# m1nty/Real-Time-Software-Defined-Radio

Measured on AMD Instinct MI355X. Metric: IQ MSamples/s through RF front-end+mono path; achieved HBM GB/s vs peak, higher is better.
Workload: dtype f32; 1 GPU; RF front end (101-tap LPF, decim 10, atan2 demod) + mono (151-tap LPF, decim 5): configs[1]+[2], one stream per GPU; block_complex=1024000, taps=101, iq=f32, parallelism=independent streams x1

## Files before the change

### real-time-software-defined-radio_amd/csrc/fe_mfma.hip

```cpp
#include <cmath>
#include <cstdlib>

#include "sdr_launch.h"

namespace {

typedef int i4v __attribute__((ext_vector_type(4)));

constexpr float kPiF = 3.14159265358979323846f;
#ifndef SDR_FE_MFMA_ABL
#define SDR_FE_MFMA_ABL 0
#endif
constexpr int kAbl = SDR_FE_MFMA_ABL;
#define SDR_FE_MFMA_WPE 3

constexpr float k2PiF = 6.28318530717958647692f;

struct MfmaFe {
  const unsigned char* iq;
  int64_t n, stride;
  int64_t M, A;
  int bps;
  int64_t total;
  const float* taps;
  float qscale;
  const float* argev;
  const i4v* afr;
  float* audio;
  int64_t audio_stride;
};

constexpr int D = 10, T = 101, TO = 256, OFF = 104;
constexpr int IMG = D * TO + 96;
constexpr int NCH = IMG / 8;
constexpr int NLD = (NCH + 63) / 64;
constexpr int TA = 151, DA = 5, AB = DA * TO, HA = 152, NW = DA * 3 + TA;
static_assert(IMG % 8 == 0 && NLD == 6, "image layout");
static_assert(D * 15 + T - 1 + (OFF - 100 - 0) < 256 && OFF - (T - 1) >= 0, "K = 256 covers the band");

__device__ __forceinline__ void lds_order() { asm volatile("" ::: "memory"); }

__device__ __forceinline__ unsigned bperm(int src_lane, unsigned v) {
  return (unsigned)__builtin_amdgcn_ds_bpermute(src_lane << 2, (int)v);
}

int tap_scale_exp(float hmax) { return (int)std::floor(std::log2((8388608.0 - 65536.0) / (double)hmax)); }

__device__ __forceinline__ int digit(int q, int k) {
  int d = 0;
  for (int j = 0; j <= k; ++j) {
    d = ((q & 0xff) ^ 0x80) - 0x80;
    q = (q - d) >> 8;
  }
  return d;
}

__device__ __forceinline__ void combine_digits(const i4v (&acc)[2][3], float (&yi)[4], float (&yq)[4]) {
#pragma unroll
  for (int i = 0; i < 4; ++i) {
    yi[i] = fmaf((float)acc[0][2][i], 65536.f, (float)(acc[0][1][i] * 256 + acc[0][0][i]));
    yq[i] = fmaf((float)acc[1][2][i], 65536.f, (float)(acc[1][1][i] * 256 + acc[1][0][i]));
  }
}
__device__ __forceinline__ f2v atan2_x2_finite(f2v y, f2v x) {
  const float ax0 = fabsf(x.x), ay0 = fabsf(y.x), ax1 = fabsf(x.y), ay1 = fabsf(y.y);
  const float mn0 = fminf(ax0, ay0), mx0 = fmaxf(ax0, ay0), mn1 = fminf(ax1, ay1), mx1 = fmaxf(ax1, ay1);
  const f2v mn = f2v{mn0, mn1};
  const f2v mxs = f2v{fmaxf(mx0, 1e-30f), fmaxf(mx1, 1e-30f)};
  const f2v rc = f2v{__builtin_amdgcn_rcpf(mxs.x), __builtin_amdgcn_rcpf(mxs.y)};
  f2v a = mn * rc;
  a = __builtin_elementwise_fma(__builtin_elementwise_fma(-mxs, a, mn), rc, a);
  const f2v s = a * a;
  auto c = [](float v) { return f2v{v, v}; };
  f2v r = c(0.002849547192454338f);
  r = __builtin_elementwise_fma(r, s, c(-0.01606736145913601f));
  r = __builtin_elementwise_fma(r, s, c(0.04268963634967804f));
  r = __builtin_elementwise_fma(r, s, c(-0.0750415101647377f));
  r = __builtin_elementwise_fma(r, s, c(0.1064087525010109f));
  r = __builtin_elementwise_fma(r, s, c(-0.1420363187789917f));
  r = __builtin_elementwise_fma(r, s, c(0.19992618262767792f));
  r = __builtin_elementwise_fma(r, s, c(-0.3333307206630707f));
  r = __builtin_elementwise_fma(r, s, c(1.0f));
  r = r * a;
  float r0 = r.x, r1 = r.y;
  r0 = (ay0 > ax0) ? 1.57079632679489662f - r0 : r0;
  r1 = (ay1 > ax1) ? 1.57079632679489662f - r1 : r1;
  r0 = (x.x < 0.f) ? 3.14159265358979324f - r0 : r0;
  r1 = (x.y < 0.f) ? 3.14159265358979324f - r1 : r1;
  asm volatile("" : "+v"(r0), "+v"(r1));
  r0 = (mx0 == 0.f) ? (__builtin_signbitf(x.x) ? 3.14159265358979324f : 0.f) : r0;
  r1 = (mx1 == 0.f) ? (__builtin_signbitf(x.y) ? 3.14159265358979324f : 0.f) : r1;
  return f2v{copysignf(r0, y.x), copysignf(r1, y.y)};
}
template <bool FINITE>
__device__ __forceinline__ void atan2_4(const float (&y)[4], const float (&x)[4], float (&phi)[4]) {
  const f2v p01 = FINITE ? atan2_x2_finite(f2v{y[0], y[1]}, f2v{x[0], x[1]}) : fast_atan2f_x2(f2v{y[0], y[1]}, f2v{x[0], x[1]});
  const f2v p23 = FINITE ? atan2_x2_finite(f2v{y[2], y[3]}, f2v{x[2], x[3]}) : fast_atan2f_x2(f2v{y[2], y[3]}, f2v{x[2], x[3]});
  phi[0] = p01.x; phi[1] = p01.y; phi[2] = p23.x; phi[3] = p23.y;
}
__device__ __forceinline__ void pk_fma_s(f2v& acc, f2v tap2, const f2v& x2) {
  asm("v_pk_fma_f32 %0, %1, %2, %0" : "+v"(acc) : "s"(tap2), "v"(x2));
}
typedef float f2a4 __attribute__((ext_vector_type(2), aligned(4)));
typedef const __attribute__((address_space(4))) float* cfp4;
typedef const __attribute__((address_space(4))) f2a4* cfp2;

__global__ __launch_bounds__(64) __attribute__((amdgpu_waves_per_eu(SDR_FE_MFMA_WPE))) void fe_mfma_mono_kernel(MfmaFe p) {
  __shared__ __attribute__((aligned(16))) signed char img[2][IMG + 16];
  __shared__ __attribute__((aligned(16))) float dh[HA + AB + 8];

  const int lane = threadIdx.x;
  const int64_t b0 = (int64_t)blockIdx.x * p.total / gridDim.x;
  const int64_t b1 = ((int64_t)blockIdx.x + 1) * p.total / gridDim.x;
  if (b0 >= b1) return;
  const int pl = lane & 15, gl = lane >> 4;

  i4v afr[4][3];
  if (p.afr != nullptr) {
#pragma unroll
    for (int ks = 0; ks < 4; ++ks)
#pragma unroll
      for (int dg = 0; dg < 3; ++dg) afr[ks][dg] = p.afr[(ks * 3 + dg) * 64 + lane];
  } else
#pragma unroll
  for (int ks = 0; ks < 4; ++ks) {
    int w[3][4] = {};
#pragma unroll
    for (int j = 0; j < 16; ++j) {
      const int k = D * pl + OFF - (64 * ks + 16 * gl + j);
      const float h = (k >= 0 && k < T) ? p.taps[k] : 0.f;
      const int q = (int)rintf(h * p.qscale);
#pragma unroll
      for (int dg = 0; dg < 3; ++dg) w[dg][j >> 2] |= (digit(q, dg) & 0xff) << (8 * (j & 3));
    }
#pragma unroll
    for (int dg = 0; dg < 3; ++dg) afr[ks][dg] = i4v{w[dg][0], w[dg][1], w[dg][2], w[dg][3]};
  }
#pragma unroll
  for (int ks = 0; ks < 4; ++ks)
#pragma unroll
    for (int dg = 0; dg < 3; ++dg) asm volatile("" : : "v"(afr[ks][dg]));
  const cfp4 gr = (cfp4)p.argev;

  f4v stg[NLD];
  const unsigned voff = 16u * lane;
  auto n_lo_of = [&](int64_t t) { return (int64_t)TO * D * t - OFF; };
  auto interior = [&](int64_t t) { return n_lo_of(t) >= 0 && n_lo_of(t) + IMG <= p.n; };
  auto base_of = [&](int s, int64_t t) { return p.iq + 2 * ((int64_t)s * p.stride + n_lo_of(t)); };
  constexpr int HC = (IMG - D * TO) / 8;
  static_assert(D * TO / 8 == 5 * 64, "5 new chunks per lane");
  auto load_image = [&](int s, int64_t t, bool halo) {
    const int cf = halo ? HC : 0;
    const unsigned char* base = base_of(s, t) + 16 * cf;
    if (kAbl & 16) return;
    static_for<0, NLD>([&](auto Q) {
      constexpr int q = Q;
      if (lane < NCH - cf - 64 * q) gload16_nt_v<0>(stg[q], voff, base + 1024 * q);
    });
  };
  auto put_chunk = [&](int c, unsigned w0, unsigned w1, unsigned w2, unsigned w3) {
    const unsigned i_lo = __builtin_amdgcn_perm(w1, w0, 0x06040200u) ^ 0x80808080u;
    const unsigned i_hi = __builtin_amdgcn_perm(w3, w2, 0x06040200u) ^ 0x80808080u;
    const unsigned q_lo = __builtin_amdgcn_perm(w1, w0, 0x07050301u) ^ 0x80808080u;
    const unsigned q_hi = __builtin_amdgcn_perm(w3, w2, 0x07050301u) ^ 0x80808080u;
    *reinterpret_cast<uint2*>(&img[0][8 * c]) = make_uint2(i_lo, i_hi);
    *reinterpret_cast<uint2*>(&img[1][8 * c]) = make_uint2(q_lo, q_hi);
  };
  auto store_image = [&](bool halo) {
    asm volatile("s_waitcnt vmcnt(0)" ::: "memory");
    const int cf = halo ? HC : 0;
    if (halo && lane < 2 * HC) {
      const int ch = lane / HC, k = lane - ch * HC;
      const uint2 v = *reinterpret_cast<const uint2*>(&img[ch][D * TO + 8 * k]);
      *reinterpret_cast<uint2*>(&img[ch][8 * k]) = v;
    }
    lds_order();
#pragma unroll
    for (int q = 0; q < NLD; ++q) {
      const int c = cf + lane + 64 * q;
      if (c < NCH) {
        asm volatile("" : "+v"(stg[q]));
        if (!(kAbl & 8))
          put_chunk(c, __float_as_uint(stg[q].x), __float_as_uint(stg[q].y), __float_as_uint(stg[q].z),
                    __float_as_uint(stg[q].w));
      }
    }
  };
  auto build_guarded = [&](int s, int64_t t) {
    const int64_t n_lo = n_lo_of(t);
    const unsigned char* base = base_of(s, t);
    for (int c = lane; c < NCH; c += 64) {
      unsigned w4[4];
#pragma unroll
      for (int e = 0; e < 4; ++e) {
        const int64_t n0 = n_lo + 8 * c + 2 * e;
        const unsigned lo = (n0 >= 0 && n0 < p.n) ? *reinterpret_cast<const unsigned short*>(base + 2 * (8 * c + 2 * e)) : 0x8080u;
        const unsigned hi = (n0 + 1 >= 0 && n0 + 1 < p.n) ? *reinterpret_cast<const unsigned short*>(base + 2 * (8 * c + 2 * e + 1)) : 0x8080u;
        w4[e] = lo | (hi << 16);
      }
      put_chunk(c, w4[0], w4[1], w4[2], w4[3]);
    }
  };

  int s = (int)(b0 / p.bps);
  int64_t t = (b0 - (int64_t)s * p.bps) * DA;
  const int64_t tps = (int64_t)p.bps * DA;
  const bool warm = t > 0;
  if (warm) --t;
  const int64_t U = (b1 - b0) * DA + (warm ? 1 : 0);
  for (int e = lane; e < HA; e += 64) dh[e] = 0.f;
  if (interior(t)) {
    load_image(s, t, false);
    store_image(false);
  } else {
    build_guarded(s, t);
  }
  auto next_s = [&](int s_, int64_t t_) { return t_ + 1 == tps ? s_ + 1 : s_; };
  auto next_t = [&](int64_t t_) { return t_ + 1 == tps ? (int64_t)0 : t_ + 1; };
  int s1 = next_s(s, t);
  int64_t t1 = next_t(t);
  float carry = 0.f;
  float d4[4] = {0.f, 0.f, 0.f, 0.f};

  constexpr int AQ = 4;
  f4v aq[AQ];
  int nq = 0;
  int qs = (int)(b0 / p.bps);
  int qj = (int)(b0 - (int64_t)qs * p.bps);
  auto queue_flush = [&]() __attribute__((always_inline)) {
    static_for<0, AQ>([&](auto K) {
      constexpr int k = K;
      if (k < nq) {
        const int64_t j = (int64_t)TO * qj + 4 * lane;
        float* ao = p.audio + (int64_t)qs * p.audio_stride + j;
        if (j + 4 <= p.A && ((uintptr_t)ao & 15) == 0) {
          *reinterpret_cast<f4v*>(ao) = aq[k];
        } else {
          const float rv[4] = {aq[k].x, aq[k].y, aq[k].z, aq[k].w};
#pragma unroll
          for (int r = 0; r < 4; ++r)
            if (j + r < p.A) ao[r] = rv[r];
        }
        if (++qj == p.bps) { qj = 0; ++qs; }
      }
    });
    nq = 0;
  };
  auto queue_put = [&](const f4v& v) __attribute__((always_inline)) {
    static_for<0, AQ>([&](auto K) {
      if ((int)K == nq) aq[K] = v;
    });
    if (++nq == AQ) queue_flush();
  };

  auto mfma_tile = [&](i4v (&acc)[2][3]) __attribute__((always_inline)) {
    lds_order();
#pragma unroll
    for (int ch = 0; ch < 2; ++ch)
#pragma unroll
      for (int dg = 0; dg < 3; ++dg) acc[ch][dg] = i4v{0, 0, 0, 0};
#pragma unroll
    for (int ks = 0; ks < 4; ++ks) {
      i4v a[3];
#pragma unroll
      for (int dg = 0; dg < 3; ++dg) a[dg] = afr[ks][dg];
      i4v bf[2];
#pragma unroll
      for (int ch = 0; ch < 2; ++ch) bf[ch] = *reinterpret_cast<const i4v*>(&img[ch][160 * pl + 64 * ks + 16 * gl]);
#pragma unroll
      for (int ch = 0; ch < 2; ++ch)
#pragma unroll
        for (int dg = 0; dg < 3; ++dg)
          acc[ch][dg] = (kAbl & 4) ? acc[ch][dg] + bf[ch]
                                   : __builtin_amdgcn_mfma_i32_16x16x64_i8(a[dg], bf[ch], acc[ch][dg], 0, 0, 0);
    }
  };
  auto epilogue = [&](const i4v (&acc)[2][3], int64_t u) __attribute__((always_inline)) {
    float yi[4], yq[4];
    combine_digits(acc, yi, yq);
    float phi[4];
    if (kAbl & 2) {
#pragma unroll
      for (int i = 0; i < 4; ++i) phi[i] = yq[i] * 1e-9f + yi[i] * 1e-9f;
    } else {
      atan2_4<true>(yq, yi, phi);
    }
    const int src = gl > 0 ? lane - 16 : (pl > 0 ? lane + 47 : 63);
    const float left = __uint_as_float(bperm(src, __float_as_uint(phi[3])));
    float prev = (lane == 0) ? carry : left;
    const int64_t mo = (int64_t)TO * t + 16 * pl + 4 * gl;
    float d[4];
#pragma unroll
    for (int i = 0; i < 4; ++i) {
      float dd = phi[i] - prev;
      if (dd > kPiF) dd -= k2PiF;
      else if (dd < -kPiF) dd += k2PiF;
      d[i] = (mo + i == 0) ? phi[i] : dd;
      prev = phi[i];
    }
    carry = __int_as_float(__builtin_amdgcn_readlane(__float_as_int(phi[3]), 63));
    const int o = 16 * pl + 4 * gl;
    const int tb = (int)(t % DA);
    if (warm && u == 0) {
      if (o >= TO - HA) *reinterpret_cast<f4v*>(&dh[HA - TO + o]) = f4v{d[0], d[1], d[2], d[3]};
    } else {
      *reinterpret_cast<f4v*>(&dh[HA + TO * tb + o]) = f4v{d[0], d[1], d[2], d[3]};
#pragma unroll
      for (int i = 0; i < 4; ++i) d4[i] = d[i];
    }
    if (!(kAbl & 1) && !(warm && u == 0) && tb == DA - 1) {
      lds_order();
      const float* aw = dh + (HA - (TA - 1)) + DA * 4 * lane;
      f2v acc[4] = {f2v{0.f, 0.f}, f2v{0.f, 0.f}, f2v{0.f, 0.f}, f2v{0.f, 0.f}};
      static_for<0, NW / 2>([&](auto W2) {
        constexpr int w = 2 * W2;
        const f2v x2 = *reinterpret_cast<const f2v*>(aw + w);
        static_for<0, 4>([&](auto RR) {
          constexpr int j = w - DA * (int)RR;
          if constexpr (j >= -1 && j <= TA - 1) {
            const f2a4 hp = *(cfp2)(gr + j);
            pk_fma_s(acc[RR], f2v{hp.x, hp.y}, x2);
          }
        });
      });
      queue_put(f4v{acc[0].x + acc[0].y, acc[1].x + acc[1].y, acc[2].x + acc[2].y, acc[3].x + acc[3].y});
      lds_order();
      if (o >= TO - HA) *reinterpret_cast<f4v*>(&dh[HA - TO + o]) = f4v{d4[0], d4[1], d4[2], d4[3]};
    }
  };
  auto advance = [&]() __attribute__((always_inline)) {
    s = s1;
    t = t1;
    if (t == 0) {
      lds_order();
      for (int e = lane; e < HA; e += 64) dh[e] = 0.f;
    }
    s1 = next_s(s, t);
    t1 = next_t(t);
  };

  bool staged = U > 1 && interior(t1);
  bool halo = staged && s1 == s && t1 == t + 1 && interior(t);
  if (staged) load_image(s1, t1, halo);
  i4v acc[2][3];
  for (int64_t u = 0; u < U; ++u) {
    const bool more = u + 1 < U;
    mfma_tile(acc);
    if (more) {
      lds_order();
      if (staged) store_image(halo);
      else build_guarded(s1, t1);
      const int s2 = next_s(s1, t1);
      const int64_t t2 = next_t(t1);
      staged = u + 2 < U && interior(t2);
      halo = staged && s2 == s1 && t2 == t1 + 1 && interior(t1);
      if (staged) load_image(s2, t2, halo);
    }
    epilogue(acc, u);
    if (more) advance();
  }
  asm volatile("s_waitcnt vmcnt(0)" ::: "memory");
  queue_flush();
}

template <int T> struct DemodShape;
template <> struct DemodShape<101> { static constexpr int KS = 4, OFF = 104; };
template <> struct DemodShape<151> { static constexpr int KS = 5, OFF = 152; };

struct MfmaDemod {
  const unsigned char* iq;
  int64_t n, stride;
  int64_t M;
  int64_t tps, total;
  const float* taps;
  float qscale;
  const i4v* afr;
  const double* zi_i;
  const double* zi_q;
  int64_t zi_stride;
  const double* prev_phase;
  float* demod;
  int64_t out_stride;
  float* last_phi;
  int* wraps;
  int vec_out;
};

__device__ inline double unwrap_step_f64_m(double dd, int* w) {
  *w = 0;
  if (fabs(dd) < 3.14159265358979323846) return dd;
  constexpr double kPi = 3.14159265358979323846, k2Pi = 6.28318530717958647692;
  double m = fmod(dd + kPi, k2Pi);
  if (m < 0) m += k2Pi;
  double ddmod = m - kPi;
  if (ddmod == -kPi && dd > 0) ddmod = kPi;
  *w = (int)llrint((ddmod - dd) / k2Pi);
  return ddmod;
}

template <int T>
__device__ __forceinline__ float output_phase(const unsigned char* iq_s, int64_t m, const float* taps, float qscale) {
  const int lane = threadIdx.x;
  int acc[2][3] = {};
  for (int k = lane; k < T; k += 64) {
    const int q = (int)rintf(taps[k] * qscale);
    const unsigned short v = *reinterpret_cast<const unsigned short*>(iq_s + 2 * (D * m - k));
    const int xi = (int)(signed char)((v & 0xff) ^ 0x80), xq = (int)(signed char)(((v >> 8) & 0xff) ^ 0x80);
#pragma unroll
    for (int dg = 0; dg < 3; ++dg) {
      const int d = digit(q, dg);
      acc[0][dg] += d * xi;
      acc[1][dg] += d * xq;
    }
  }
#pragma unroll
  for (int ch = 0; ch < 2; ++ch)
#pragma unroll
    for (int dg = 0; dg < 3; ++dg) acc[ch][dg] = wave_sum_i(acc[ch][dg]);
  const float yi = fmaf((float)acc[0][2], 65536.f, (float)(acc[0][1] * 256 + acc[0][0]));
  const float yq = fmaf((float)acc[1][2], 65536.f, (float)(acc[1][1] * 256 + acc[1][0]));
  return fast_atan2f_x2(f2v{yq, yq}, f2v{yi, yi}).x;
}

template <int T>
__global__ __launch_bounds__(64) void fe_mfma_demod_kernel(MfmaDemod p) {
  constexpr int KS = DemodShape<T>::KS, OFF = DemodShape<T>::OFF, K = 64 * KS;
  constexpr int IM = 160 * 15 + K;
  constexpr int NC = IM / 8, NL = (NC + 63) / 64;
  static_assert(IM % 8 == 0 && OFF % 8 == 0 && OFF >= T - 1 && D * 15 + OFF <= K - 1, "image / band layout");
  __shared__ __attribute__((aligned(16))) signed char img[2][IM + 16];

  const int lane = threadIdx.x;
  const int64_t b0 = (int64_t)blockIdx.x * p.total / gridDim.x;
  const int64_t b1 = ((int64_t)blockIdx.x + 1) * p.total / gridDim.x;
  if (b0 >= b1) return;
  const int pl = lane & 15, gl = lane >> 4;

  i4v afr[KS][3];
  if (p.afr != nullptr) {
#pragma unroll
    for (int ks = 0; ks < KS; ++ks)
#pragma unroll
      for (int dg = 0; dg < 3; ++dg) afr[ks][dg] = p.afr[(ks * 3 + dg) * 64 + lane];
  } else
#pragma unroll
  for (int ks = 0; ks < KS; ++ks) {
    int w[3][4] = {};
#pragma unroll
    for (int j = 0; j < 16; ++j) {
      const int k = D * pl + OFF - (64 * ks + 16 * gl + j);
      const float h = (k >= 0 && k < T) ? p.taps[k] : 0.f;
      const int q = (int)rintf(h * p.qscale);
#pragma unroll
      for (int dg = 0; dg < 3; ++dg) w[dg][j >> 2] |= (digit(q, dg) & 0xff) << (8 * (j & 3));
    }
#pragma unroll
    for (int dg = 0; dg < 3; ++dg) afr[ks][dg] = i4v{w[dg][0], w[dg][1], w[dg][2], w[dg][3]};
  }
#pragma unroll
  for (int ks = 0; ks < KS; ++ks)
#pragma unroll
    for (int dg = 0; dg < 3; ++dg) asm volatile("" : : "v"(afr[ks][dg]));

  f4v stg[NL];
  const unsigned voff = 16u * lane;
  auto n_lo_of = [&](int64_t t) { return (int64_t)TO * D * t - OFF; };
  auto interior = [&](int64_t t) { return n_lo_of(t) >= 0 && n_lo_of(t) + IM <= p.n; };
  auto base_of = [&](int s, int64_t t) { return p.iq + 2 * ((int64_t)s * p.stride + n_lo_of(t)); };
  constexpr int HC = (IM - D * TO) / 8;
  static_assert(D * TO / 8 == 5 * 64, "5 new chunks per lane");
  auto load_image = [&](int s, int64_t t, bool halo) {
    const int cf = halo ? HC : 0;
    const unsigned char* base = base_of(s, t) + 16 * cf;
    static_for<0, NL>([&](auto Q) {
      constexpr int q = Q;
      if (lane < NC - cf - 64 * q) gload16_nt_v<0>(stg[q], voff, base + 1024 * q);
    });
  };
  auto put_chunk = [&](int c, unsigned w0, unsigned w1, unsigned w2, unsigned w3) {
    const unsigned i_lo = __builtin_amdgcn_perm(w1, w0, 0x06040200u) ^ 0x80808080u;
    const unsigned i_hi = __builtin_amdgcn_perm(w3, w2, 0x06040200u) ^ 0x80808080u;
    const unsigned q_lo = __builtin_amdgcn_perm(w1, w0, 0x07050301u) ^ 0x80808080u;
    const unsigned q_hi = __builtin_amdgcn_perm(w3, w2, 0x07050301u) ^ 0x80808080u;
    *reinterpret_cast<uint2*>(&img[0][8 * c]) = make_uint2(i_lo, i_hi);
    *reinterpret_cast<uint2*>(&img[1][8 * c]) = make_uint2(q_lo, q_hi);
  };
  bool st1 = false;
  auto store_image = [&](bool halo) {
    if (__builtin_amdgcn_readfirstlane((int)st1)) asm volatile("s_waitcnt vmcnt(1)" ::: "memory");
    else asm volatile("s_waitcnt vmcnt(0)" ::: "memory");
    const int cf = halo ? HC : 0;
    if (halo && lane < 2 * HC) {
      const int ch = lane / HC, k = lane - ch * HC;
      const uint2 v = *reinterpret_cast<const uint2*>(&img[ch][D * TO + 8 * k]);
      *reinterpret_cast<uint2*>(&img[ch][8 * k]) = v;
    }
    lds_order();
#pragma unroll
    for (int q = 0; q < NL; ++q) {
      const int c = cf + lane + 64 * q;
      if (c < NC) {
        asm volatile("" : "+v"(stg[q]));
        put_chunk(c, __float_as_uint(stg[q].x), __float_as_uint(stg[q].y), __float_as_uint(stg[q].z),
                  __float_as_uint(stg[q].w));
      }
    }
  };
  auto build_guarded = [&](int s, int64_t t) {
    const int64_t n_lo = n_lo_of(t);
    const unsigned char* base = base_of(s, t);
    for (int c = lane; c < NC; c += 64) {
      unsigned w4[4];
#pragma unroll
      for (int e = 0; e < 4; ++e) {
        const int64_t n0 = n_lo + 8 * c + 2 * e;
        const unsigned lo = (n0 >= 0 && n0 < p.n) ? *reinterpret_cast<const unsigned short*>(base + 2 * (8 * c + 2 * e)) : 0x8080u;
        const unsigned hi = (n0 + 1 >= 0 && n0 + 1 < p.n) ? *reinterpret_cast<const unsigned short*>(base + 2 * (8 * c + 2 * e + 1)) : 0x8080u;
        w4[e] = lo | (hi << 16);
      }
      put_chunk(c, w4[0], w4[1], w4[2], w4[3]);
    }
  };

  int s = (int)(b0 / p.tps);
  int64_t t = b0 - (int64_t)s * p.tps;
  const int64_t U = b1 - b0;
  float carry = t > 0 ? output_phase<T>(p.iq + 2 * (int64_t)s * p.stride, TO * t - 1, p.taps, p.qscale) : 0.f;
  if (interior(t)) {
    load_image(s, t, false);
    store_image(false);
  } else {
    build_guarded(s, t);
  }
  int s_nx = s;
  int64_t t_nx = t + 1;
  if (t_nx == p.tps) { t_nx = 0; ++s_nx; }
  int wsum = 0;
  const double zscale = (double)p.qscale * 128.0;

  bool staged = U > 1 && interior(t_nx);
  bool halo = staged && s_nx == s && t_nx == t + 1 && interior(t);
  if (staged) load_image(s_nx, t_nx, halo);
  for (int64_t u = 0; u < U; ++u) {
    const bool more = u + 1 < U;
    lds_order();
    i4v acc[2][3];
#pragma unroll
    for (int ch = 0; ch < 2; ++ch)
#pragma unroll
      for (int dg = 0; dg < 3; ++dg) acc[ch][dg] = i4v{0, 0, 0, 0};
#pragma unroll
    for (int ks = 0; ks < KS; ++ks) {
      i4v bf[2];
#pragma unroll
      for (int ch = 0; ch < 2; ++ch) bf[ch] = *reinterpret_cast<const i4v*>(&img[ch][160 * pl + 64 * ks + 16 * gl]);
#pragma unroll
      for (int ch = 0; ch < 2; ++ch)
#pragma unroll
        for (int dg = 0; dg < 3; ++dg)
          acc[ch][dg] = __builtin_amdgcn_mfma_i32_16x16x64_i8(afr[ks][dg], bf[ch], acc[ch][dg], 0, 0, 0);
    }
    if (more) {
      lds_order();
      if (staged) store_image(halo);
      else build_guarded(s_nx, t_nx);
      int s2 = s_nx;
      int64_t t2 = t_nx + 1;
      if (t2 == p.tps) { t2 = 0; ++s2; }
      staged = u + 2 < U && interior(t2);
      halo = staged && s2 == s_nx && t2 == t_nx + 1 && interior(t_nx);
      if (staged) load_image(s2, t2, halo);
    }
    const int64_t mo = (int64_t)TO * t + 16 * pl + 4 * gl;
    float yi[4], yq[4];
    combine_digits(acc, yi, yq);
    if (t == 0 && p.zi_i != nullptr) {
#pragma unroll
      for (int i = 0; i < 4; ++i)
        if (D * (mo + i) < T - 1) {
          yi[i] += (float)(p.zi_i[(int64_t)s * p.zi_stride + D * (mo + i)] * zscale);
          yq[i] += (float)(p.zi_q[(int64_t)s * p.zi_stride + D * (mo + i)] * zscale);
        }
    }
    float phi[4];
    atan2_4<false>(yq, yi, phi);
    const int src = gl > 0 ? lane - 16 : (pl > 0 ? lane + 47 : 63);
    const float left = __uint_as_float(bperm(src, __float_as_uint(phi[3])));
    float prev = (lane == 0) ? carry : left;
    constexpr bool keep = true;
    float d[4];
#pragma unroll
    for (int i = 0; i < 4; ++i) {
      const int64_t m = mo + i;
      int wk = 0;
      if (m == 0) {
        const double ps = p.prev_phase ? p.prev_phase[s] : 0.0;
        d[i] = (float)unwrap_step_f64_m((double)phi[i] - ps, &wk);
      } else {
        float dd = phi[i] - prev;
        if (dd > kPiF) { dd -= k2PiF; wk = -1; }
        else if (dd < -kPiF) { dd += k2PiF; wk = 1; }
        d[i] = dd;
      }
      if (keep && m < p.M) wsum += wk;
      prev = phi[i];
    }
    carry = __int_as_float(__builtin_amdgcn_readlane(__float_as_int(phi[3]), 63));
    if (keep) {
      float* out = p.demod + (int64_t)s * p.out_stride + mo;
      if (p.vec_out && mo + 4 <= p.M) {
        *reinterpret_cast<f4v*>(out) = f4v{d[0], d[1], d[2], d[3]};
      } else {
#pragma unroll
        for (int i = 0; i < 4; ++i)
          if (mo + i < p.M) out[i] = d[i];
      }
      if (p.last_phi != nullptr) {
#pragma unroll
        for (int i = 0; i < 4; ++i)
          if (mo + i == p.M - 1) p.last_phi[s] = phi[i];
      }
    }
    const bool wr = keep && (!more || s_nx != s) && p.wraps != nullptr;
    if (wr) {
      const int w = wave_sum_i(wsum);
      if (lane == 0 && w != 0) atomicAdd(p.wraps + s, w);
      wsum = 0;
    }
    st1 = keep && p.vec_out && t > 0 && (int64_t)TO * t + TO < p.M && !wr;
    if (more) {
      s = s_nx;
      t = t_nx;
      t_nx = t + 1;
      s_nx = s;
      if (t_nx == p.tps) { t_nx = 0; ++s_nx; }
    }
  }
}

template <int T>
hipError_t launch_demod_mfma_t(const FeLaunch& a, hipStream_t st) {
  float hmax = 0.f;
  for (int k = 0; k < T; ++k) hmax = std::max(hmax, std::fabs(a.taps->h[k]));
  if (!(hmax > 0.f) || !std::isfinite(hmax)) return hipErrorInvalidValue;
  const int S = tap_scale_exp(hmax);
  MfmaDemod p{};
  p.iq = static_cast<const unsigned char*>(a.iq);
  p.n = a.n;
  p.stride = a.nstreams > 1 ? a.stride : 0;
  p.M = (a.n + D - 1) / D;
  p.tps = (p.M + TO - 1) / TO;
  p.total = p.tps * a.nstreams;
  if (p.total > 0x7fffffff) return hipErrorInvalidValue;
  p.taps = a.taps_dev;
  p.qscale = std::ldexp(1.0f, S);
  p.afr = reinterpret_cast<const i4v*>(a.afr);
  p.zi_i = a.zi_i;
  p.zi_q = a.zi_q;
  p.zi_stride = a.zi_stride;
  p.prev_phase = a.prev_phase;
  p.demod = a.demod;
  p.out_stride = a.out_stride;
  p.last_phi = a.last_phi;
  p.wraps = a.wraps;
  p.vec_out = ((a.out_stride % 4) == 0 && ((uintptr_t)a.demod % 16) == 0) ? 1 : 0;
  static std::atomic<int> slot_cache[kMaxDevices];
  const int slots = per_device(slot_cache, [] {
    int per = 0;
    if (hipOccupancyMaxActiveBlocksPerMultiprocessor(&per, fe_mfma_demod_kernel<T>, 64, 0) != hipSuccess || per <= 0) per = 1;
    return device_cus() * std::min(per, 12);
  });
  const int64_t run = std::max<int64_t>(1, (p.total + slots - 1) / slots);
  const int64_t grid = std::max<int64_t>(1, (p.total + run - 1) / run);
  hipLaunchKernelGGL(fe_mfma_demod_kernel<T>, dim3((unsigned)grid), dim3(64), 0, st, p);
  return hipGetLastError();
}

}

bool sdr_mfma_fragments(const float* h, int T_, std::vector<int>* out) {
  int KS, OFFT;
  if (T_ == 101) { KS = DemodShape<101>::KS; OFFT = DemodShape<101>::OFF; }
  else if (T_ == 151) { KS = DemodShape<151>::KS; OFFT = DemodShape<151>::OFF; }
  else return false;
  static_assert(DemodShape<101>::KS == 4 && DemodShape<101>::OFF == OFF, "mono and demod kernels share the T = 101 shape");
  float hmax = 0.f;
  for (int k = 0; k < T_; ++k) hmax = std::max(hmax, std::fabs(h[k]));
  if (!(hmax > 0.f) || !std::isfinite(hmax)) return false;
  const float qs = std::ldexp(1.0f, tap_scale_exp(hmax));
  out->assign((size_t)KS * 3 * 64 * 4, 0);
  for (int ks = 0; ks < KS; ++ks)
    for (int lane = 0; lane < 64; ++lane) {
      const int pl = lane & 15, gl = lane >> 4;
      for (int j = 0; j < 16; ++j) {
        const int k = D * pl + OFFT - (64 * ks + 16 * gl + j);
        const float hv = (k >= 0 && k < T_) ? h[k] : 0.f;
        int q = (int)std::rint(hv * qs);
        for (int dg = 0; dg < 3; ++dg) {
          const int d = ((q & 0xff) ^ 0x80) - 0x80;
          q = (q - d) >> 8;
          (*out)[(((size_t)ks * 3 + dg) * 64 + lane) * 4 + (j >> 2)] |= (d & 0xff) << (8 * (j & 3));
        }
      }
    }
  return true;
}

hipError_t sdr_launch_fe_mfma(const FeLaunch& a, hipStream_t st) {
  if (!a.u8 || a.D != D || a.hist != 0 || a.i_ds || a.q_ds || a.demod == nullptr) return hipErrorInvalidValue;
  if (((uintptr_t)a.iq & 15) != 0 || (a.nstreams > 1 && (a.stride % 8) != 0)) return hipErrorInvalidValue;
  if (a.n <= 0 || a.nstreams <= 0) return hipSuccess;
  if (a.T == 101) return launch_demod_mfma_t<101>(a, st);
  if (a.T == 151) return launch_demod_mfma_t<151>(a, st);
  return hipErrorInvalidValue;
}

hipError_t sdr_launch_fe_mono_mfma(const FeLaunch& a, const float* ataps_rev, int TA_, int DA_, float* audio,
                                   int64_t audio_stride, hipStream_t st) {
  if (!a.u8 || a.D != D || a.T != T || TA_ != TA || DA_ != DA || a.hist != 0 || a.zi_i || a.prev_phase || a.demod ||
      a.i_ds || a.last_phi || a.wraps)
    return hipErrorInvalidValue;
  if (((uintptr_t)a.iq & 15) != 0 || (a.nstreams > 1 && (a.stride % 8) != 0)) return hipErrorInvalidValue;
  if (a.n <= 0 || a.nstreams <= 0) return hipSuccess;
  float hmax = 0.f;
  for (int k = 0; k < T; ++k) hmax = std::max(hmax, std::fabs(a.taps->h[k]));
  if (!(hmax > 0.f) || !std::isfinite(hmax)) return hipErrorInvalidValue;
  const int S = tap_scale_exp(hmax);
  MfmaFe p{};
  p.iq = static_cast<const unsigned char*>(a.iq);
  p.n = a.n;
  p.stride = a.nstreams > 1 ? a.stride : 0;
  p.M = (a.n + D - 1) / D;
  p.A = (p.M + DA - 1) / DA;
  p.bps = (int)((p.M + AB - 1) / AB);
  p.total = (int64_t)p.bps * a.nstreams;
  if (p.total > 0x7fffffff) return hipErrorInvalidValue;
  p.taps = a.taps_dev;
  p.qscale = std::ldexp(1.0f, S);
  p.afr = reinterpret_cast<const i4v*>(a.afr);
  p.argev = ataps_rev;
  p.audio = audio;
  p.audio_stride = audio_stride;
  static std::atomic<int> slot_cache[kMaxDevices];
  const int slots = per_device(slot_cache, [] {
    int per = 0;
    if (hipOccupancyMaxActiveBlocksPerMultiprocessor(&per, fe_mfma_mono_kernel, 64, 0) != hipSuccess || per <= 0) per = 1;
    const int cap = 4 * SDR_FE_MFMA_WPE;
    return device_cus() * std::min(per, cap);
  });

  const int64_t grid = std::min<int64_t>(slots, p.total);
  hipLaunchKernelGGL(fe_mfma_mono_kernel, dim3((unsigned)grid), dim3(64), 0, st, p);
  return hipGetLastError();
}
```

Measured before the change: 738,200 MS/s.

## Run mono audio FIR on MFMA with split-f16 and pack waves per block

Replaces the scalar packed-FMA 151-tap audio filter with 16x16x32 f16 MFMA ops. Both data and taps are split into hi/lo halves, and the result is rebuilt with three MFMAs per K-step so it keeps close to f32 accuracy. The delay history moves to f16 hi/lo LDS buffers, and the audio tap fragments are built once per block into shared memory. The launch changes from one-wave blocks to 12-wave blocks, each wave handling an independent virtual work slice. This raises LDS use per block, and the split-f16 trick carries some precision risk.

```diff
diff --git a/real-time-software-defined-radio_amd/csrc/fe_mfma.hip b/real-time-software-defined-radio_amd/csrc/fe_mfma.hip
--- a/real-time-software-defined-radio_amd/csrc/fe_mfma.hip
+++ b/real-time-software-defined-radio_amd/csrc/fe_mfma.hip
@@ -2,6 +2,7 @@
 #include <cstdlib>
 
 #include "sdr_launch.h"
+#include "sdr_mma.h"
 
 namespace {
 
@@ -13,6 +14,7 @@
 #endif
 constexpr int kAbl = SDR_FE_MFMA_ABL;
 #define SDR_FE_MFMA_WPE 3
+#define SDR_FE_MFMA_NWV (4 * SDR_FE_MFMA_WPE)
 
 constexpr float k2PiF = 6.28318530717958647692f;
 
@@ -22,6 +24,7 @@
   int64_t M, A;
   int bps;
   int64_t total;
+  int64_t nv;
   const float* taps;
   float qscale;
   const float* argev;
@@ -34,7 +37,8 @@
 constexpr int IMG = D * TO + 96;
 constexpr int NCH = IMG / 8;
 constexpr int NLD = (NCH + 63) / 64;
-constexpr int TA = 151, DA = 5, AB = DA * TO, HA = 152, NW = DA * 3 + TA;
+constexpr int TA = 151, DA = 5, AB = DA * TO, HA = 152;
+constexpr int AKS = 8, PL = 80 * 15 + 32 * AKS;
 static_assert(IMG % 8 == 0 && NLD == 6, "image layout");
 static_assert(D * 15 + T - 1 + (OFF - 100 - 0) < 256 && OFF - (T - 1) >= 0, "K = 256 covers the band");
 
@@ -98,20 +102,38 @@
   const f2v p23 = FINITE ? atan2_x2_finite(f2v{y[2], y[3]}, f2v{x[2], x[3]}) : fast_atan2f_x2(f2v{y[2], y[3]}, f2v{x[2], x[3]});
   phi[0] = p01.x; phi[1] = p01.y; phi[2] = p23.x; phi[3] = p23.y;
 }
-__device__ __forceinline__ void pk_fma_s(f2v& acc, f2v tap2, const f2v& x2) {
-  asm("v_pk_fma_f32 %0, %1, %2, %0" : "+v"(acc) : "s"(tap2), "v"(x2));
-}
-typedef float f2a4 __attribute__((ext_vector_type(2), aligned(4)));
-typedef const __attribute__((address_space(4))) float* cfp4;
-typedef const __attribute__((address_space(4))) f2a4* cfp2;
-
-__global__ __launch_bounds__(64) __attribute__((amdgpu_waves_per_eu(SDR_FE_MFMA_WPE))) void fe_mfma_mono_kernel(MfmaFe p) {
-  __shared__ __attribute__((aligned(16))) signed char img[2][IMG + 16];
-  __shared__ __attribute__((aligned(16))) float dh[HA + AB + 8];
-
-  const int lane = threadIdx.x;
-  const int64_t b0 = (int64_t)blockIdx.x * p.total / gridDim.x;
-  const int64_t b1 = ((int64_t)blockIdx.x + 1) * p.total / gridDim.x;
+
+__global__ __launch_bounds__(64 * SDR_FE_MFMA_NWV) __attribute__((amdgpu_waves_per_eu(SDR_FE_MFMA_WPE))) void fe_mfma_mono_kernel(MfmaFe p) {
+  constexpr int NWV = SDR_FE_MFMA_NWV;
+  __shared__ __attribute__((aligned(16))) signed char img_s[NWV][2][IMG + 16];
+  __shared__ __attribute__((aligned(16))) _Float16 dp_s[NWV][2][PL];
+  __shared__ __attribute__((aligned(16))) h8v aaf[2][AKS][64];
+
+  if (!(kAbl & 1))
+    for (int idx = threadIdx.x; idx < AKS * 64; idx += 64 * NWV) {
+      const int st = idx >> 6, ln = idx & 63, bb = ln & 15, gg = ln >> 4;
+      h8v hi, lo;
+#pragma unroll
+      for (int e = 0; e < 8; ++e) {
+        const int k = DA * bb + HA - (32 * st + 8 * gg + e);
+        const MmHL hl = mm_split((k >= 0 && k < TA) ? p.argev[TA - 1 - k] : 0.f);
+        hi[e] = hl.hi;
+        lo[e] = hl.lo;
+      }
+      aaf[0][st][ln] = hi;
+      aaf[1][st][ln] = lo;
+    }
+  __syncthreads();
+
+  const int wv = __builtin_amdgcn_readfirstlane((int)(threadIdx.x >> 6));
+  signed char (&img)[2][IMG + 16] = img_s[wv];
+  _Float16* const dph = dp_s[wv][0];
+  _Float16* const dpl = dp_s[wv][1];
+  const int lane = threadIdx.x & 63;
+  const int64_t v = (int64_t)wv * gridDim.x + blockIdx.x;
+  if (v >= p.nv) return;
+  const int64_t b0 = v * p.total / p.nv;
+  const int64_t b1 = (v + 1) * p.total / p.nv;
   if (b0 >= b1) return;
   const int pl = lane & 15, gl = lane >> 4;
 
@@ -140,7 +162,6 @@
   for (int ks = 0; ks < 4; ++ks)
 #pragma unroll
     for (int dg = 0; dg < 3; ++dg) asm volatile("" : : "v"(afr[ks][dg]));
-  const cfp4 gr = (cfp4)p.argev;
 
   f4v stg[NLD];
   const unsigned voff = 16u * lane;
@@ -208,7 +229,9 @@
   const bool warm = t > 0;
   if (warm) --t;
   const int64_t U = (b1 - b0) * DA + (warm ? 1 : 0);
-  for (int e = lane; e < HA; e += 64) dh[e] = 0.f;
+  const _Float16 hz = (_Float16)0.f;
+  for (int e = lane; e < HA; e += 64) dph[e] = dpl[e] = hz;
+  for (int e = HA + AB + lane; e < PL; e += 64) dph[e] = dpl[e] = hz;
   if (interior(t)) {
     load_image(s, t, false);
     store_image(false);
@@ -220,7 +243,6 @@
   int s1 = next_s(s, t);
   int64_t t1 = next_t(t);
   float carry = 0.f;
-  float d4[4] = {0.f, 0.f, 0.f, 0.f};
 
   constexpr int AQ = 4;
   f4v aq[AQ];
@@ -231,7 +253,7 @@
     static_for<0, AQ>([&](auto K) {
       constexpr int k = K;
       if (k < nq) {
-        const int64_t j = (int64_t)TO * qj + 4 * lane;
+        const int64_t j = (int64_t)TO * qj + 16 * pl + 4 * gl;
         float* ao = p.audio + (int64_t)qs * p.audio_stride + j;
         if (j + 4 <= p.A && ((uintptr_t)ao & 15) == 0) {
           *reinterpret_cast<f4v*>(ao) = aq[k];
@@ -301,31 +323,37 @@
     carry = __int_as_float(__builtin_amdgcn_readlane(__float_as_int(phi[3]), 63));
     const int o = 16 * pl + 4 * gl;
     const int tb = (int)(t % DA);
-    if (warm && u == 0) {
-      if (o >= TO - HA) *reinterpret_cast<f4v*>(&dh[HA - TO + o]) = f4v{d[0], d[1], d[2], d[3]};
-    } else {
-      *reinterpret_cast<f4v*>(&dh[HA + TO * tb + o]) = f4v{d[0], d[1], d[2], d[3]};
-#pragma unroll
-      for (int i = 0; i < 4; ++i) d4[i] = d[i];
-    }
-    if (!(kAbl & 1) && !(warm && u == 0) && tb == DA - 1) {
+    h4v hv, lv;
+    mm_split4(make_float4(d[0], d[1], d[2], d[3]), &hv, &lv);
+    const bool wu = warm && u == 0;
+    if (!wu || o >= TO - HA) {
+      const int q = wu ? HA - TO + o : HA + TO * tb + o;
+      *reinterpret_cast<h4v*>(dph + q) = hv;
+      *reinterpret_cast<h4v*>(dpl + q) = lv;
+    }
+    if (!(kAbl & 1) && !wu && tb == DA - 1) {
       lds_order();
-      const float* aw = dh + (HA - (TA - 1)) + DA * 4 * lane;
-      f2v acc[4] = {f2v{0.f, 0.f}, f2v{0.f, 0.f}, f2v{0.f, 0.f}, f2v{0.f, 0.f}};
-      static_for<0, NW / 2>([&](auto W2) {
-        constexpr int w = 2 * W2;
-        const f2v x2 = *reinterpret_cast<const f2v*>(aw + w);
-        static_for<0, 4>([&](auto RR) {
-          constexpr int j = w - DA * (int)RR;
-          if constexpr (j >= -1 && j <= TA - 1) {
-            const f2a4 hp = *(cfp2)(gr + j);
-            pk_fma_s(acc[RR], f2v{hp.x, hp.y}, x2);
-          }
-        });
+      f4v acc_h = f4v{0.f, 0.f, 0.f, 0.f}, acc_c = acc_h;
+      static_for<0, AKS>([&](auto ST) {
+        constexpr int st = ST;
+        const int uu = 80 * pl + 32 * st + 8 * gl;
+        const h8v xh = *reinterpret_cast<const h8v*>(dph + uu);
+        const h8v xl = *reinterpret_cast<const h8v*>(dpl + uu);
+        const h8v ah = aaf[0][st][lane];
+        const h8v al = aaf[1][st][lane];
+        acc_h = __builtin_amdgcn_mfma_f32_16x16x32_f16(ah, xh, acc_h, 0, 0, 0);
+        acc_c = __builtin_amdgcn_mfma_f32_16x16x32_f16(ah, xl, acc_c, 0, 0, 0);
+        acc_c = __builtin_amdgcn_mfma_f32_16x16x32_f16(al, xh, acc_c, 0, 0, 0);
       });
-      queue_put(f4v{acc[0].x + acc[0].y, acc[1].x + acc[1].y, acc[2].x + acc[2].y, acc[3].x + acc[3].y});
+      f4v y;
+#pragma unroll
+      for (int r = 0; r < 4; ++r) y[r] = fmaf(acc_c[r], 1.f / MM_LO, acc_h[r]);
+      queue_put(y);
       lds_order();
-      if (o >= TO - HA) *reinterpret_cast<f4v*>(&dh[HA - TO + o]) = f4v{d4[0], d4[1], d4[2], d4[3]};
+      if (o >= TO - HA) {
+        *reinterpret_cast<h4v*>(dph + HA - TO + o) = hv;
+        *reinterpret_cast<h4v*>(dpl + HA - TO + o) = lv;
+      }
     }
   };
   auto advance = [&]() __attribute__((always_inline)) {
@@ -333,7 +361,7 @@
     t = t1;
     if (t == 0) {
       lds_order();
-      for (int e = lane; e < HA; e += 64) dh[e] = 0.f;
+      for (int e = lane; e < HA; e += 64) dph[e] = dpl[e] = hz;
     }
     s1 = next_s(s, t);
     t1 = next_t(t);
@@ -744,12 +772,12 @@
   static std::atomic<int> slot_cache[kMaxDevices];
   const int slots = per_device(slot_cache, [] {
     int per = 0;
-    if (hipOccupancyMaxActiveBlocksPerMultiprocessor(&per, fe_mfma_mono_kernel, 64, 0) != hipSuccess || per <= 0) per = 1;
-    const int cap = 4 * SDR_FE_MFMA_WPE;
+    if (hipOccupancyMaxActiveBlocksPerMultiprocessor(&per, fe_mfma_mono_kernel, 64 * SDR_FE_MFMA_NWV, 0) != hipSuccess || per <= 0) per = 1;
+    const int cap = 4 * SDR_FE_MFMA_WPE / SDR_FE_MFMA_NWV;
     return device_cus() * std::min(per, cap);
   });
-
-  const int64_t grid = std::min<int64_t>(slots, p.total);
-  hipLaunchKernelGGL(fe_mfma_mono_kernel, dim3((unsigned)grid), dim3(64), 0, st, p);
+  p.nv = std::min<int64_t>((int64_t)slots * SDR_FE_MFMA_NWV, p.total);
+  const int64_t grid = std::min<int64_t>(slots, p.nv);
+  hipLaunchKernelGGL(fe_mfma_mono_kernel, dim3((unsigned)grid), dim3(64 * SDR_FE_MFMA_NWV), 0, st, p);
   return hipGetLastError();
 }
```

After: 737,700 MS/s. About the same (-0.1%).
